# OFA-Sys/OFASys

Hardware: AMD Instinct MI355X
Metric: multimodal tokens/sec (enc+dec train step) (higher is better)
Workload: dtype bf16

## Files before the change

### ofasys_amd/csrc/gemm_mfma.hip

```cpp
#include <mutex>
#include <utility>
#include <vector>

#include "gemm_core.h"

namespace ofa {


#ifdef OFA_GEMM_TIMELINE
#define OFA_TL(i) do { if (threadIdx.x == 0 && (i) < 24) tl[i] = __builtin_amdgcn_s_memtime(); } while (0)
#define OFA_TL_BEGIN                                                                                                           \
  unsigned long long* tl = (unsigned long long*)ws + 32 * (blockIdx.x + gridDim.x * (blockIdx.y + gridDim.y * blockIdx.z));   \
  int tlk = 8;                                                                                                                 \
  if (threadIdx.x == 0) {                                                                                                      \
    tl[5] = __builtin_amdgcn_s_getreg((31 << 11) | 4);                                                                         \
    tl[6] = __builtin_amdgcn_s_getreg((31 << 11) | 20);                                                                        \
    tl[7] = __builtin_amdgcn_s_memrealtime();                                                                                  \
  }                                                                                                                            \
  OFA_TL(0)
#define OFA_TL_STEP do { OFA_TL(tlk); ++tlk; } while (0)
#define OFA_TL_END                                                        \
  do {                                                                    \
    OFA_TL(3);                                                            \
    asm volatile("s_waitcnt vmcnt(0)" ::: "memory");                      \
// ... 229 lines not shown
  const int tid = threadIdx.x, lane = tid & 63, wave = tid >> 6;
  const int wm = wave / WN, wn = wave % WN;
  const int ntiles = tiles_m * tiles_n;
  int t, ks;
  tile_and_slice(ntiles, t, ks);
  constexpr int GM = 8;
  const int gsz = GM * tiles_n;
  const int gid = t / gsz, first_m = gid * GM;
  const int rows_in_group = (tiles_m - first_m) < GM ? (tiles_m - first_m) : GM;
  const int tm = first_m + (t % gsz) % rows_in_group, tn = (t % gsz) / rows_in_group;
  const int m0 = tm * BM, n0 = tn * BN;
  const int bz = blockIdx.z;
  const bf16_t* A = (const bf16_t*)g.A + batch_off(bz, g.batch_inner, g.strideA, g.strideA2);
  const bf16_t* B = (const bf16_t*)g.B + batch_off(bz, g.batch_inner, g.strideB, g.strideB2);
  const int kbeg = ks * ksplit;
  const int kend = (kbeg + ksplit < g.K) ? kbeg + ksplit : g.K;
  const int nk = (kend - kbeg) / BK;

  f32x16 acc[TMW][TNW];
#pragma unroll
  for (int i = 0; i < TMW; ++i)
#pragma unroll
    for (int j = 0; j < TNW; ++j)
#pragma unroll
      for (int r = 0; r < 16; ++r) acc[i][j][r] = 0.f;

  const int wave_u = __builtin_amdgcn_readfirstlane(wave);
  const bf16_t* pa[NVA];
  const bf16_t* pb[NVB];
  glds_ptrs<BM, A_KMAJ, NT, NVA, true>(pa, A, g.lda, m0, g.M, kbeg, tid, g.a_krows);
  glds_ptrs<BN, B_KMAJ, NT, NVB>(pb, B, g.ldb, n0, g.N, kbeg, tid, g.b_krows);
  const int64_t stepA = A_KMAJ ? BK : (int64_t)BK * g.lda, stepB = B_KMAJ ? BK : (int64_t)BK * g.ldb;
  int knext = kbeg;
  auto dma = [&](int stage) {
    if (!A_KMAJ && knext + BK > g.a_krows)
      glds_ptrs<BM, A_KMAJ, NT, NVA, true>(pa, A, g.lda, m0, g.M, knext, tid, g.a_krows);
    if (!B_KMAJ && knext + BK > g.b_krows)
      glds_ptrs<BN, B_KMAJ, NT, NVB>(pb, B, g.ldb, n0, g.N, knext, tid, g.b_krows);
    bf16_t* st = reinterpret_cast<bf16_t*>(smem_raw + (size_t)stage * STG);
    glds_issue<NT, NVA>(pa, stepA, st, wave_u);
    glds_issue<NT, NVB>(pb, stepB, st + EA, wave_u);
    knext += BK;
  };
  int issued = 0;
  for (; issued < S - 1 && issued < nk; ++issued) dma(issued);

  const uint32_t lds0 = (uint32_t)(uintptr_t)smem_raw;
  FragAddr<BM, A_KMAJ> fax[TMW];
  FragAddr<BN, B_KMAJ> faw[TNW];
#pragma unroll
  for (int i = 0; i < TMW; ++i) fax[i].init(lds0, wm * 32 * TMW + i * 32, lane);
#pragma unroll
  for (int j = 0; j < TNW; ++j) faw[j].init(lds0 + (uint32_t)EA * 2u, wn * 32 * TNW + j * 32, lane);
  constexpr int NA = A_KMAJ ? 4 : 1, NB = B_KMAJ ? 4 : 1;
  int stage = 0;
  for (int kt = 0; kt < nk; ++kt) {
    const int later = issued - kt - 1;
    if (S >= 4 && later >= 2) asm volatile("s_waitcnt vmcnt(%0)" ::"n"(2 * P) : "memory");
    else if (later >= 1) asm volatile("s_waitcnt vmcnt(%0)" ::"n"(P) : "memory");
    else asm volatile("s_waitcnt vmcnt(0)" ::: "memory");
    __builtin_amdgcn_sched_barrier(0);
    __builtin_amdgcn_s_barrier();
    __builtin_amdgcn_sched_barrier(0);
    const bool refill = issued < nk;
    bf16_t* rst = reinterpret_cast<bf16_t*>(smem_raw + (size_t)((stage + S - 1) % S) * STG);
    if (refill && !A_KMAJ && knext + BK > g.a_krows)
      glds_ptrs<BM, A_KMAJ, NT, NVA, true>(pa, A, g.lda, m0, g.M, knext, tid, g.a_krows);
    if (refill && !B_KMAJ && knext + BK > g.b_krows)
      glds_ptrs<BN, B_KMAJ, NT, NVB>(pb, B, g.ldb, n0, g.N, knext, tid, g.b_krows);
    u64x2 x0[TMW], w0[TNW], x1[TMW], w1[TNW];
#define RING_ISSUE(KK, X, W)                                                                                           \
    static_for<0, TMW>([&](auto ic) { frag_issue<BM, A_KMAJ, KK, 0>(X[decltype(ic)::value], fax[decltype(ic)::value]); }); \
    static_for<0, TNW>([&](auto jc) { frag_issue<BN, B_KMAJ, KK, 0>(W[decltype(jc)::value], faw[decltype(jc)::value]); })
#define RING_WAIT(X, W)                                                                                                \
    if constexpr (TMW == 2 && TNW == 2) asm volatile("s_waitcnt lgkmcnt(0)" : "+v"(X[0]), "+v"(X[TMW - 1]), "+v"(W[0]), "+v"(W[TNW - 1])); \
    else if constexpr (TMW == 1 && TNW == 2) asm volatile("s_waitcnt lgkmcnt(0)" : "+v"(X[0]), "+v"(W[0]), "+v"(W[TNW - 1]));            \
    else if constexpr (TMW == 2 && TNW == 1) asm volatile("s_waitcnt lgkmcnt(0)" : "+v"(X[0]), "+v"(X[TMW - 1]), "+v"(W[0]));            \
    else { static_assert(TMW <= 2 && TNW <= 2, "RING_WAIT names every fragment register: add the shape");              \
           asm volatile("s_waitcnt lgkmcnt(0)" : "+v"(X[0]), "+v"(W[0])); }
#define RING_MMA(X, W)                                                                                                 \
    _Pragma("unroll") for (int i = 0; i < TMW; ++i) _Pragma("unroll") for (int j = 0; j < TNW; ++j)                    \
        acc[i][j] = mfma16<F16>(W[j], X[i], acc[i][j])
#define RING_DMA(Q)                                                                                                    \
    __builtin_amdgcn_sched_barrier(0);                                                                                 \
    if (refill) {                                                                                                      \
      static_for<(Q) * P / 4, ((Q) + 1) * P / 4>([&](auto pc) {                                                        \
        constexpr int pi = decltype(pc)::value;                                                                        \
        if constexpr (pi < NVA) {                                                                                      \
          __builtin_amdgcn_global_load_lds((gvoid_t*)pa[pi], (lvoid_t*)(rst + (wave_u * 64 + pi * NT) * 8), 16, 0, 0); \
          pa[pi] += stepA;                                                                                             \
        } else {                                                                                                       \
          __builtin_amdgcn_global_load_lds((gvoid_t*)pb[pi - NVA], (lvoid_t*)(rst + EA + (wave_u * 64 + (pi - NVA) * NT) * 8), 16, 0, 0); \
          pb[pi - NVA] += stepB;                                                                                       \
        }                                                                                                              \
      });                                                                                                              \
    }                                                                                                                  \
    __builtin_amdgcn_sched_barrier(0)
    RING_ISSUE(0, x0, w0);
    RING_WAIT(x0, w0);
    RING_ISSUE(1, x1, w1);
    RING_MMA(x0, w0);
    RING_DMA(0);
    RING_WAIT(x1, w1);
    RING_ISSUE(2, x0, w0);
    RING_MMA(x1, w1);
    RING_DMA(1);
    RING_WAIT(x0, w0);
    RING_ISSUE(3, x1, w1);
    RING_MMA(x0, w0);
    RING_DMA(2);
    RING_WAIT(x1, w1);
    RING_MMA(x1, w1);
    RING_DMA(3);
    if (refill) {
      knext += BK;
      ++issued;
    }
#undef RING_DMA
#undef RING_ISSUE
#undef RING_WAIT
#undef RING_MMA
    const bool wrap = stage == S - 1;
    const uint32_t delta = wrap ? (uint32_t)(0u - (uint32_t)(S - 1) * STG) : STG;
#pragma unroll
    for (int i = 0; i < TMW; ++i)
#pragma unroll
      for (int q = 0; q < NA; ++q) fax[i].a[q] += delta;
#pragma unroll
    for (int j = 0; j < TNW; ++j)
#pragma unroll
      for (int q = 0; q < NB; ++q) faw[j].a[q] += delta;
    stage = wrap ? 0 : stage + 1;
  }
  __syncthreads();
  {
    const bool split = gridDim.y > 1;
    constexpr int REGION = ((int)(S * STG) / (WM * WN)) & ~1023;
    unsigned char* wl = smem_raw + wave * REGION;
    const int m_w = m0 + wm * 32 * TMW, n_w = n0 + wn * 32 * TNW;
    if (split) {
      const int64_t n4 = (g.N + 3) & ~3;
      float* wsb = ws + ((int64_t)bz * gridDim.y + ks) * g.M * n4;
      epilogue_lds<TMW, TNW, true, true, F16>(g, acc, wl, REGION, wsb, n4, m_w, n_w, lane);
    } else {
      const int64_t coff = batch_off(bz, g.batch_inner, g.strideC, g.strideC2);
      void* Cb = OUT_F32 ? (void*)((float*)g.C + coff) : (void*)((bf16_t*)g.C + coff);
      epilogue_lds<TMW, TNW, OUT_F32, false, F16>(g, acc, wl, REGION, Cb, g.ldc, m_w, n_w, lane);
    }
  }
}



template <int TM, int TN, bool A_KMAJ, bool B_KMAJ, bool OUT_F32, int WGM, int WGN, bool F16>
__device__ __forceinline__ void gemm_big_body(const GemmArgs& g, int tiles_m, int tiles_n, int ksplit,
                                              float* __restrict__ ws, int t, int ks, int bz, int nsplit, bool to_ws) {
  constexpr int BM = 32 * TM * WGM, BN = 32 * TN * WGN, NT = 64 * WGM * WGN;
  static_assert(BM <= 256 && BN <= 256, "operand stage is 256 rows");
  static_assert(A_KMAJ || BM == 256, "m-major tiles are 256 wide (swizzle)");
  static_assert(B_KMAJ || BN == 256, "m-major tiles are 256 wide (swizzle)");
  constexpr int NVA = BM * 8 / NT, NVB = BN * 8 / NT;
  constexpr int STAGE = 256 * BK;
  extern __shared__ __attribute__((aligned(16))) unsigned char smem_raw[];
  bf16_t* sA0 = reinterpret_cast<bf16_t*>(smem_raw);
  bf16_t* sA1 = sA0 + STAGE;
  bf16_t* sB0 = sA1 + STAGE;
  bf16_t* sB1 = sB0 + STAGE;

  const int tid = threadIdx.x, lane = tid & 63, wave = tid >> 6;
  const int wm = wave / WGN, wn = wave % WGN;
  OFA_TL_BEGIN;
  constexpr int GM = 8;
  const int gsz = GM * tiles_n;
  const int gid = t / gsz, first_m = gid * GM;
  const int rows_in_group = (tiles_m - first_m) < GM ? (tiles_m - first_m) : GM;
  const int tm = first_m + (t % gsz) % rows_in_group, tn = (t % gsz) / rows_in_group;
  const int m0 = tm * BM, n0 = tn * BN;
  const bf16_t* A = (const bf16_t*)g.A + batch_off(bz, g.batch_inner, g.strideA, g.strideA2);
  const bf16_t* B = (const bf16_t*)g.B + batch_off(bz, g.batch_inner, g.strideB, g.strideB2);
  const int kbeg = ks * ksplit;
  const int kend = (kbeg + ksplit < g.K) ? kbeg + ksplit : g.K;
  const int nk = (kend - kbeg) / BK;

  f32x16 acc[TM][TN];
#pragma unroll
  for (int i = 0; i < TM; ++i)
#pragma unroll
    for (int j = 0; j < TN; ++j)
#pragma unroll
      for (int r = 0; r < 16; ++r) acc[i][j][r] = 0.f;

  const int wave_u = __builtin_amdgcn_readfirstlane(wave);
  const bf16_t* pa[NVA];
  const bf16_t* pb[NVB];
  glds_ptrs<BM, A_KMAJ, NT, NVA, true>(pa, A, g.lda, m0, g.M, kbeg, tid, g.a_krows);
  glds_ptrs<BN, B_KMAJ, NT, NVB>(pb, B, g.ldb, n0, g.N, kbeg, tid, g.b_krows);
  const int64_t stepA = A_KMAJ ? BK : (int64_t)BK * g.lda, stepB = B_KMAJ ? BK : (int64_t)BK * g.ldb;
  int knext = kbeg;
  auto dma = [&](bf16_t* da, bf16_t* db) {
    if (!A_KMAJ && knext + BK > g.a_krows)
      glds_ptrs<BM, A_KMAJ, NT, NVA, true>(pa, A, g.lda, m0, g.M, knext, tid, g.a_krows);
    if (!B_KMAJ && knext + BK > g.b_krows)
      glds_ptrs<BN, B_KMAJ, NT, NVB>(pb, B, g.ldb, n0, g.N, knext, tid, g.b_krows);
    glds_issue<NT, NVA>(pa, stepA, da, wave_u);
    glds_issue<NT, NVB>(pb, stepB, db, wave_u);
    knext += BK;
  };
  const uint32_t lds0 = (uint32_t)(uintptr_t)smem_raw;
  BigAddr<BM, A_KMAJ> fax;
  BigAddr<BN, B_KMAJ> faw;
  fax.init(lds0, wm * TM * 32, lane);
  faw.init(lds0 + 2 * STAGE * 2, wn * TN * 32, lane);

  u64x2 xa[2][TM], wb[2][TN];
#ifndef OFA_BIG_RPG_TN
#define OFA_BIG_RPG_TN 1
#endif
  constexpr int RPG = (!A_KMAJ && !B_KMAJ) ? OFA_BIG_RPG_TN : 1;
#define BIG_ISSUE(KK, SET)                                                                                        \
  static_for<0, TM>([&](auto ic) { big_frag<BM, A_KMAJ, KK, decltype(ic)::value, 0>(xa[SET][decltype(ic)::value], fax); }); \
  static_for<0, TN>([&](auto ic) { big_frag<BN, B_KMAJ, KK, decltype(ic)::value, 0>(wb[SET][decltype(ic)::value], faw); })
#define BIG_WAITCNT "s_waitcnt lgkmcnt(0)"
#define BIG_WAIT(SET)                                                                  \
  if constexpr (TM == 4 && TN == 2)                                                    \
    asm volatile(BIG_WAITCNT : "+v"(xa[SET][0]), "+v"(xa[SET][1]), "+v"(xa[SET][2]), "+v"(xa[SET][3]),   \
                 "+v"(wb[SET][0]), "+v"(wb[SET][TN - 1]));                                                          \
  else if constexpr (TM == 3 && TN == 2)                                               \
    asm volatile(BIG_WAITCNT : "+v"(xa[SET][0]), "+v"(xa[SET][1]), "+v"(xa[SET][2]),                     \
                 "+v"(wb[SET][0]), "+v"(wb[SET][TN - 1]));                                                          \
  else if constexpr (TM == 4 && TN == 4)                                               \
    asm volatile(BIG_WAITCNT : "+v"(xa[SET][0]), "+v"(xa[SET][1]), "+v"(xa[SET][2]), "+v"(xa[SET][3]),   \
                 "+v"(wb[SET][0]), "+v"(wb[SET][1]), "+v"(wb[SET][2]), "+v"(wb[SET][TN - 1]));                      \
  else                                                                                 \
    static_assert(TM == 4 && TN == 2, "BIG_WAIT names every fragment register: add the shape")
#define BIG_SB __builtin_amdgcn_sched_barrier(0)
#define BIG_SLICE(SET, KKN)                                                                                         \
  static_for<0, TM * TN>([&](auto tc) {                                                                             \
    constexpr int t = decltype(tc)::value, i = t / TN, j = t % TN;                                                  \
    acc[i][j] = mfma16<F16>(wb[SET][j], xa[SET][i], acc[i][j]); \
    static_for<0, RPG>([&](auto qc) {                                                                               \
      constexpr int r = big_read_after(t * RPG + decltype(qc)::value, TM + TN);                                     \
      if constexpr (r >= 0 && r < TM) big_frag<BM, A_KMAJ, KKN, (r < TM ? r : 0), 0>(xa[1 - (SET)][r < TM ? r : 0], fax); \
      if constexpr (r >= TM) big_frag<BN, B_KMAJ, KKN, (r >= TM ? r - TM : 0), 0>(wb[1 - (SET)][r >= TM ? r - TM : 0], faw); \
    });                                                                                                             \
    BIG_SB;                                                                                                         \
  })
  if (nk > 0) {
    dma(sA0, sB0);
    asm volatile("s_waitcnt vmcnt(0)" ::: "memory");
    __syncthreads();
    OFA_TL(1);
    if (nk > 1) dma(sA1, sB1);
    BIG_ISSUE(0, 0);
    bf16_t* curA = sA0;
    bf16_t* curB = sB0;
    for (int kt = 0; kt < nk; ++kt) {
      BIG_WAIT(0); BIG_SB; BIG_SLICE(0, 1);
      BIG_WAIT(1); BIG_SB; BIG_SLICE(1, 2);
      BIG_WAIT(0); BIG_SB; BIG_SLICE(0, 3);
      BIG_WAIT(1);
      if (kt + 1 < nk) {
        asm volatile("s_waitcnt vmcnt(0)" ::: "memory");
        __syncthreads();
      }
      const bool more2 = kt + 2 < nk;
      if (more2 && !A_KMAJ && knext + BK > g.a_krows)
        glds_ptrs<BM, A_KMAJ, NT, NVA, true>(pa, A, g.lda, m0, g.M, knext, tid, g.a_krows);
      if (more2 && !B_KMAJ && knext + BK > g.b_krows)
        glds_ptrs<BN, B_KMAJ, NT, NVB>(pb, B, g.ldb, n0, g.N, knext, tid, g.b_krows);
#pragma unroll
      for (int i = 0; i < 4; ++i) {
        fax.a[i] ^= (uint32_t)(STAGE * 2);
        faw.a[i] ^= (uint32_t)(STAGE * 2);
      }
      BIG_SB;
      static_for<0, TM * TN>([&](auto tc) {
        constexpr int t = decltype(tc)::value, i = t / TN, j = t % TN;
        acc[i][j] = mfma16<F16>(wb[1][j], xa[1][i], acc[i][j]);
        static_for<0, RPG>([&](auto qc) {
          constexpr int r = big_read_after(t * RPG + decltype(qc)::value, TM + TN);
          if constexpr (r >= 0 && r < TM) big_frag<BM, A_KMAJ, 0, (r < TM ? r : 0), 0>(xa[0][r < TM ? r : 0], fax);
          if constexpr (r >= TM) big_frag<BN, B_KMAJ, 0, (r >= TM ? r - TM : 0), 0>(wb[0][r >= TM ? r - TM : 0], faw);
        });
        if (more2) {
          constexpr int NP = NVA + NVB, NM = TM * TN;
          static_for<t * NP / NM, (t + 1) * NP / NM>([&](auto pc) {
            constexpr int pi = decltype(pc)::value;
            if constexpr (pi < NVA) {
              __builtin_amdgcn_global_load_lds((gvoid_t*)pa[pi], (lvoid_t*)(curA + (wave_u * 64 + pi * NT) * 8), 16, 0, 0);
              pa[pi] += stepA;
            } else {
              __builtin_amdgcn_global_load_lds((gvoid_t*)pb[pi - NVA], (lvoid_t*)(curB + (wave_u * 64 + (pi - NVA) * NT) * 8), 16, 0, 0);
              pb[pi - NVA] += stepB;
            }
          });
        }
        BIG_SB;
      });
      if (more2) knext += BK;
      OFA_TL_STEP;
      curA = (bf16_t*)((uintptr_t)curA ^ (uintptr_t)(STAGE * 2));
      curB = (bf16_t*)((uintptr_t)curB ^ (uintptr_t)(STAGE * 2));
    }
    BIG_WAIT(0);
  }
#undef BIG_SLICE
#undef BIG_SB
#undef BIG_WAIT
#undef BIG_ISSUE
  __syncthreads();
  OFA_TL(2);
  {
    const bool split = to_ws || nsplit > 1;
    constexpr int REGION = 4 * STAGE * 2 / (WGM * WGN);
    unsigned char* wl = smem_raw + wave * REGION;
    const int m_w = m0 + wm * TM * 32, n_w = n0 + wn * TN * 32;
    if (split) {
      const int64_t n4 = (g.N + 3) & ~3;
      float* wsb = ws + ((int64_t)bz * nsplit + ks) * g.M * n4;
      epilogue_lds<TM, TN, true, true, F16>(g, acc, wl, REGION, wsb, n4, m_w, n_w, lane);
    } else {
      const int64_t coff = batch_off(bz, g.batch_inner, g.strideC, g.strideC2);
      void* Cb = OUT_F32 ? (void*)((float*)g.C + coff) : (void*)((bf16_t*)g.C + coff);
      epilogue_lds<TM, TN, OUT_F32, false, F16>(g, acc, wl, REGION, Cb, g.ldc, m_w, n_w, lane);
    }
  }
  OFA_TL_END;
}

template <int TM, int TN, bool A_KMAJ, bool B_KMAJ, bool OUT_F32, int WGM = 2, int WGN = 2, bool F16 = false>
__global__ __launch_bounds__(64 * WGM * WGN) void gemm_big_kernel(GemmArgs g, int tiles_m, int tiles_n, int ksplit,
                                                                 float* __restrict__ ws) {
  int t, ks;
  tile_and_slice(tiles_m * tiles_n, t, ks);
  gemm_big_body<TM, TN, A_KMAJ, B_KMAJ, OUT_F32, WGM, WGN, F16>(g, tiles_m, tiles_n, ksplit, ws, t, ks, (int)blockIdx.z,
                                                                (int)gridDim.y, false);
}

template <bool B_KMAJ, bool OUT_F32, bool F16>
__global__ __launch_bounds__(512) void gemm_big_mixed_kernel(GemmArgs g, int tiles_n, int rows_big, int rows_small) {
  const int nbig = rows_big * tiles_n, nsmall = rows_small * tiles_n;
  const int xcd = blockIdx.x & 7, local = blockIdx.x >> 3;
  auto lo = [](int n, int x) { const int q = n >> 3, r = n & 7; return x < r ? x * (q + 1) : r * (q + 1) + (x - r) * q; };
  const int b0 = lo(nbig, xcd), nb = lo(nbig, xcd + 1) - b0, s0 = lo(nsmall, xcd), ns = lo(nsmall, xcd + 1) - s0;
  if (local < nb) {
    gemm_big_body<4, 2, true, B_KMAJ, OUT_F32, 2, 4, F16>(g, rows_big, tiles_n, g.K, nullptr, b0 + local, 0, 0, 1, false);
  } else if (local - nb < ns) {
    const int64_t r0 = (int64_t)rows_big * 256;
    g.A = (const bf16_t*)g.A + r0 * g.lda;
    g.C = OUT_F32 ? (void*)((float*)g.C + r0 * g.ldc) : (void*)((bf16_t*)g.C + r0 * g.ldc);
    g.M -= (int)r0;
    gemm_big_body<3, 2, true, B_KMAJ, OUT_F32, 2, 4, F16>(g, rows_small, tiles_n, g.K, nullptr, s0 + local - nb, 0, 0, 1, false);
  }
}

struct TileTime {
  int slots;
  double step, step_nt, per_tile;
  double tile_us(int nk, bool nt) const { return nk * (nt ? step_nt : step) + per_tile; }
  double us(int64_t tiles, int nk, bool nt) const { return (double)cdiv(tiles, slots) * tile_us(nk, nt); }
};
constexpr TileTime TT_128{512, 0.90, 1.0, 4.2}, TT_256{256, 1.45, 1.45, 7.6}, TT_192{256, 1.13, 1.13, 6.5};

static double mixed_time_us(int nbig, int nsmall, int nk) {
  const double t4 = TT_256.tile_us(nk, false), t3 = TT_192.tile_us(nk, false);
  double worst = 0.0;
  for (int x = 0; x < 8; ++x) {
    auto lo = [](int n, int x_) { const int q = n >> 3, r = n & 7; return x_ < r ? x_ * (q + 1) : r * (q + 1) + (x_ - r) * q; };
    const int nb = lo(nbig, x + 1) - lo(nbig, x), ns = lo(nsmall, x + 1) - lo(nsmall, x);
    double cu[32];
    for (int c = 0; c < 32; ++c) cu[c] = 0.0;
    for (int i = 0; i < nb + ns; ++i) {
      int best = 0;
      for (int c = 1; c < 32; ++c) best = cu[c] < cu[best] ? c : best;
      cu[best] += i < nb ? t4 : t3;
    }
    for (int c = 0; c < 32; ++c) worst = cu[c] > worst ? cu[c] : worst;
  }
  return worst;
}

constexpr int BIG_LDS = 4 * 256 * BK * sizeof(bf16_t);

bool gemm_lds_attr(const void* kern, int bytes, uint64_t& done) {
  int dev = 0;
  if (hipGetDevice(&dev) != hipSuccess || dev < 0 || dev >= 64) return false;
  if (done >> dev & 1) return true;
  if (hipFuncSetAttribute(kern, hipFuncAttributeMaxDynamicSharedMemorySize, bytes) != hipSuccess) {
    (void)hipGetLastError();
    return false;
  }
  done |= 1ull << dev;
  return true;
}

template <bool BKM, bool OF, bool F16>
static bool launch_big_mixed(const GemmArgs& g, int rows_big, int rows_small, hipStream_t st) {
  const int tiles_n = cdiv(g.N, 256), nbig = rows_big * tiles_n, nsmall = rows_small * tiles_n;
  auto kern = gemm_big_mixed_kernel<BKM, OF, F16>;
  static uint64_t attr_done = 0;
  if (!gemm_lds_attr((const void*)kern, BIG_LDS, attr_done)) return false;
  const int per_xcd = cdiv(nbig, 8) + cdiv(nsmall, 8);
  hipLaunchKernelGGL(kern, dim3(8 * per_xcd), dim3(512), BIG_LDS, st, g, tiles_n, rows_big, rows_small);
  return true;
}


template <bool F16, bool = false>
__global__ __launch_bounds__(512) void gemm_group_tn_kernel(GroupArgs ga) {
  GemmArgs g;
  int t, ks;
  const GroupItem* itp = group_enter(ga, g, t, ks);
  if (!itp) return;
  const GroupItem& it = *itp;
  gemm_big_body<4, 2, false, false, false, 2, 4, F16>(g, it.tiles_m, it.tiles_n, it.ksplit, it.ws, t, ks, 0, it.splits, it.out == nullptr);
}

template <bool OUT_F32, bool F16 = false>
__global__ __launch_bounds__(256) void splitk_reduce_kernel(GemmArgs g, const float* __restrict__ ws, int splits) {
  const int64_t quads = (int64_t)g.M * ((g.N + 3) / 4);
  const int bz = blockIdx.y;
  const int64_t coff = batch_off(bz, g.batch_inner, g.strideC, g.strideC2);
  void* Cb = OUT_F32 ? (void*)((float*)g.C + coff) : (void*)((bf16_t*)g.C + coff);
  for (int64_t i = (int64_t)blockIdx.x * blockDim.x + threadIdx.x; i < quads; i += (int64_t)gridDim.x * blockDim.x) {
    const int m = (int)(i / ((g.N + 3) / 4)), n = (int)(i % ((g.N + 3) / 4)) * 4;
    float4 s = make_float4(0.f, 0.f, 0.f, 0.f);
    for (int k = 0; k < splits; ++k) {
      const float4 p = *reinterpret_cast<const float4*>(ws + (((int64_t)bz * splits + k) * g.M + m) * ((g.N + 3) & ~3) + n);
      s.x += p.x; s.y += p.y; s.z += p.z; s.w += p.w;
    }
    epilogue_store<OUT_F32, F16>(g, Cb, m, n, s.x, s.y, s.z, s.w);
  }
}

bool gemm_mfma_supported(const GemmArgs& g) {
  if (g.M <= 0 || g.N <= 0 || g.K <= 0) return false;
  const int64_t M8 = (g.M + 7) & ~7, N8 = (g.N + 7) & ~7, N4 = (g.N + 3) & ~3, K8 = (g.K + 7) & ~7;
  if ((g.lda & 7) || (g.ldb & 7) || (g.ldc & 3) || N4 > g.ldc) return false;
  if ((g.strideA & 7) || (g.strideB & 7) || (g.strideC & 3)) return false;
  if ((g.strideA2 & 7) || (g.strideB2 & 7) || (g.strideC2 & 3)) return false;
  if (!g.transA && (g.K & 7)) {
    if (g.transB || !(g.flags & OFA_GEMM_A_KPAD_ZERO) || K8 > g.lda) return false;
  }
  if (g.transB && (g.K & 7)) return false;
  if (g.transA && M8 > g.lda) return false;
  if (!g.transB && N8 > g.ldb) return false;
  if ((g.flags & OFA_GEMM_BIAS_COL) && (g.N & 3)) return false;
  if (((uintptr_t)g.A & 15) || ((uintptr_t)g.B & 15) || ((uintptr_t)g.C & 15)) return false;
  if ((g.flags & OFA_GEMM_BIAS_COL) && ((uintptr_t)g.bias & 7)) return false;
  return true;
}

struct GemmPlan {
  int kernel;
  int wm, wn;
  int tm, tn;
  int splits, ksplit, K;
  int mixed_a, mixed_b;
  int colstat_rows;
  bool reduce;
  int pp;
  int bm() const { return 32 * tm * wm; }
  int bn() const { return 32 * tn * wn; }
};

struct PlanKnobs {
  int tile = 0;
  int pp = -1;
  int mixed = -1;
  int split_min_k = 2048;
};

static PlanKnobs plan_knobs() {
  PlanKnobs k;
#ifdef OFA_DEBUG_SWITCHES
  auto env = [](const char* name, int dflt) { const char* e = getenv(name); return e ? atoi(e) : dflt; };
  static const int split_min_k = env("OFA_GEMM_SPLIT_MIN_K", k.split_min_k);
  k = PlanKnobs{env("OFA_GEMM_TILE", k.tile), env("OFA_GEMM_PP", k.pp), env("OFA_GEMM_MIXED", k.mixed), split_min_k};
#endif
  return k;
}

static int pp_variant(const PlanKnobs& kn, bool trans_a, bool trans_b, int K) {
  if (kn.pp >= 0) return kn.pp;
  if (trans_a && !trans_b) return 23;
  if (!trans_a && !trans_b && K >= 2048) return 23;
  return 0;
}

static GemmPlan gemm_plan(GemmArgs g, int batch, bool has_ws, int64_t ws_bytes, const PlanKnobs& kn) {
  if ((g.flags & OFA_GEMM_A_KPAD_ZERO) && !g.transA && !g.transB && (g.K % BK) != 0 && ((g.K + BK - 1) / BK) * BK <= g.lda)
    g.K = ((g.K + BK - 1) / BK) * BK;
  if (g.transA && !g.transB && (g.K % BK) != 0 && !(g.flags & OFA_GEMM_NO_LDS_DMA)) g.K = ((g.K + BK - 1) / BK) * BK;
  const bool dma = (g.K % BK) == 0 && !(g.flags & OFA_GEMM_NO_LDS_DMA);
  const int64_t t22 = (int64_t)cdiv(g.M, 128) * cdiv(g.N, 128) * batch;
  const int64_t t12 = (int64_t)cdiv(g.M, 64) * cdiv(g.N, 128) * batch;
  const int64_t t11 = (int64_t)cdiv(g.M, 64) * cdiv(g.N, 64) * batch;
  int maxs = has_ws ? g.K / 256 : 1;
  maxs = maxs < 1 ? 1 : (maxs > 32 ? 32 : maxs);
  if (g.K < kn.split_min_k || t22 >= 256) maxs = 1;
  if (!g.transA && g.K <= 4096 && t11 >= 256) maxs = 1;
  const int64_t want = 384;
  int wm, wn;
  int64_t tiles;
  if (t22 * maxs >= want && g.M > 64 && g.N >= 128) { wm = 2; wn = 2; tiles = t22; }
  else if (t12 * maxs >= want && g.N >= 128) { wm = 1; wn = 2; tiles = t12; }
  else { wm = 1; wn = 1; tiles = t11; }
  if (kn.tile == 22) { wm = 2; wn = 2; tiles = t22; }
  else if (kn.tile == 12) { wm = 1; wn = 2; tiles = t12; }
  else if (kn.tile == 11) { wm = 1; wn = 1; tiles = t11; }
  int big_tm = 0;
  const bool big_ok = dma && g.N >= 256 && g.M >= 192;
  const bool forced_small = kn.tile == 22 || kn.tile == 12 || kn.tile == 11;
  const int nk = g.K / BK;
  const int64_t t4 = (int64_t)cdiv(g.M, 256) * cdiv(g.N, 256) * batch, t3 = (int64_t)cdiv(g.M, 192) * cdiv(g.N, 256) * batch;
  if (big_ok && !forced_small) {
    if (kn.tile == 44 || kn.tile == 84) big_tm = 4;
    else if (kn.tile == 34 || kn.tile == 83) big_tm = g.transA ? 4 : 3;
    else if (!g.transA) {
      if (batch == 1 && nk >= 4 && t22 >= 512 && wm == 2 && wn == 2) {
        const double e2 = TT_128.us(t22, nk, g.transB);
        const double e4 = t4 >= 128 ? TT_256.us(t4, nk, false) : 1e30, e3 = t3 >= 128 ? TT_192.us(t3, nk, false) : 1e30;
        if (e4 <= e3 && e4 < 0.95 * e2) big_tm = 4;
        else if (e3 < e4 && e3 < 0.95 * e2) big_tm = 3;
      }
    } else {
      const double f4 = (double)t4 / (double)(cdiv(t4, 256) * 256) * ((double)g.M / (cdiv(g.M, 256) * 256)) * ((double)g.N / (cdiv(g.N, 256) * 256));
      if (f4 >= 0.7 && (g.K >= 1024 || t4 <= 256)) big_tm = 4;
    }
    if (big_tm) tiles = big_tm == 4 ? t4 : t3;
  }
  int splits = 1;
  if (!big_tm && big_ok && !kn.tile && !g.transA && batch == 1 && has_ws && g.K >= 8192) {
    int s = t4 <= 64 ? (int)(256 / t4) : 1;
    s = s > maxs ? maxs : s;
    while (s > 1 && (int64_t)s * g.M * ((g.N + 3) & ~3) * 4 > ws_bytes) --s;
    if (s >= 4) {
      big_tm = 4;
      tiles = t4;
      splits = s;
    }
  }
  if (!big_tm && tiles < want && maxs > 1) {
    splits = (int)((want + tiles - 1) / tiles);
    if (splits > maxs) splits = maxs;
    while (splits > 1 && (int64_t)splits * batch * g.M * ((g.N + 3) & ~3) * 4 > ws_bytes) --splits;
  }
  int ksplit = g.K;
  if (splits > 1) {
    ksplit = cdiv(cdiv(g.K, splits), BK) * BK;
    splits = cdiv(g.K, ksplit);
  }
  GemmPlan p{};
  p.splits = splits;
  p.ksplit = ksplit;
  p.K = g.K;
  p.reduce = splits > 1 && !(g.flags & OFA_GEMM_DEFER_REDUCE);
  if (big_tm) {
    p.wm = 2; p.wn = 4; p.tm = big_tm; p.tn = 2;
    p.pp = pp_variant(kn, g.transA, g.transB, g.K);
    p.kernel = p.pp && !(g.flags & OFA_GEMM_OUT_F32) && !(g.transA && g.transB) ? OFA_GEMM_KERNEL_PP : OFA_GEMM_KERNEL_BIG;
  } else if (dma && (int64_t)cdiv(g.M, 64 * wm) * cdiv(g.N, 64 * wn) * splits * batch <= ((wm == 1 && wn == 1) ? 512 : 256) &&
             ksplit >= 4 * BK) {
    p.kernel = OFA_GEMM_KERNEL_RING;
    p.wm = 2; p.wn = 2; p.tm = wm; p.tn = wn;
  } else {
    p.kernel = dma ? OFA_GEMM_KERNEL_LDS_DMA : OFA_GEMM_KERNEL_REG;
    p.wm = wm; p.wn = wn; p.tm = 2; p.tn = 2;
  }
  p.colstat_rows = splits > 1 || batch != 1 ? 0 : 32 * p.tm;
  if (kn.mixed != 0 && big_ok && !kn.tile && !g.transA && batch == 1 && splits == 1 && !g.colstat && !(g.flags & OFA_GEMM_BIAS_ROW) &&
      g.M >= 1024 && g.N >= 512 && g.K >= 4 * BK && pp_variant(kn, false, g.transB != 0, g.K) == 0) {
    struct Key { int M, N, K, tb; };
    struct Val { int a, b; double t; };
    static std::mutex mu;
    static std::vector<std::pair<Key, Val>> cache;
    const int tiles_n = cdiv(g.N, 256);
    Val best{0, 0, 1e30};
    bool hit = false;
    {
      std::lock_guard<std::mutex> lk(mu);
      for (auto& e : cache)
        if (e.first.M == g.M && e.first.N == g.N && e.first.K == g.K && e.first.tb == g.transB) { best = e.second; hit = true; break; }
    }
    if (!hit) {
      const int amax = g.M / 256;
      for (int a = 1; a <= amax; ++a) {
        const int rest = g.M - a * 256;
        if (rest <= 0) break;
        const int b = cdiv(rest, 192);
        const double t = mixed_time_us(a * tiles_n, b * tiles_n, nk);
        if (t < best.t) best = Val{a, b, t};
      }
      std::lock_guard<std::mutex> lk(mu);
      if (cache.size() < 256) cache.push_back({Key{g.M, g.N, g.K, g.transB}, best});
    }
    const bool modelled = (wm == 2 && wn == 2) || big_tm;
    const double cur = big_tm == 4 ? TT_256.us(tiles, nk, false) : big_tm == 3 ? TT_192.us(tiles, nk, false) : TT_128.us(tiles, nk, g.transB);
    if (best.a > 0 && best.b > 0 && (kn.mixed == 1 || (modelled && best.t < 0.95 * cur))) {
      p.kernel = OFA_GEMM_KERNEL_MIXED;
      p.wm = 2; p.wn = 4; p.tm = 4; p.tn = 2;
      p.mixed_a = best.a;
      p.mixed_b = best.b;
    }
  }
  return p;
}

template <auto KERN>
static void launch_tiles(int lds, const GemmArgs& g, int batch, const GemmPlan& p, float* ws, hipStream_t st) {
  static uint64_t attr_done = 0;
  (void)gemm_lds_attr((const void*)KERN, lds, attr_done);
  const int tiles_m = cdiv(g.M, p.bm()), tiles_n = cdiv(g.N, p.bn());
  hipLaunchKernelGGL(KERN, dim3(tiles_m * tiles_n, p.splits, batch), dim3(64 * p.wm * p.wn), lds, st, g, tiles_m, tiles_n, p.ksplit, ws);
}

template <int WM, int WN, bool AK, bool BKM, bool OF, bool F16>
static void launch_cfg2(const GemmArgs& g, int batch, const GemmPlan& p, float* ws, hipStream_t st) {
  constexpr int BM = 64 * WM, BN = 64 * WN;
  if (p.kernel == OFA_GEMM_KERNEL_LDS_DMA)
    launch_tiles<gemm_mfma_kernel<WM, WN, AK, BKM, OF, true, F16>>(2 * (BM + BN) * BK * sizeof(bf16_t), g, batch, p, ws, st);
  else
    launch_tiles<gemm_mfma_kernel<WM, WN, AK, BKM, OF, false, F16>>(2 * (TileGeom<BM, AK>::ELEMS + TileGeom<BN, BKM>::ELEMS) * sizeof(bf16_t),
                                                                    g, batch, p, ws, st);
}

template <bool AK, bool BKM, bool OF, bool F16>
static int launch_plan(const GemmArgs& g, int batch, const GemmPlan& p, float* ws, hipStream_t st) {
  switch (p.kernel) {
    case OFA_GEMM_KERNEL_PP:
      if (gemm_pp_launch(p.pp, g, batch, p.tm, p.splits, p.ksplit, ws, st, F16)) break;
      [[fallthrough]];
    case OFA_GEMM_KERNEL_BIG:
      if constexpr (AK) {
        if (p.tm == 3) { launch_tiles<gemm_big_kernel<3, 2, AK, BKM, OF, 2, 4, F16>>(BIG_LDS, g, batch, p, ws, st); break; }
      }
      launch_tiles<gemm_big_kernel<4, 2, AK, BKM, OF, 2, 4, F16>>(BIG_LDS, g, batch, p, ws, st);
      break;
    case OFA_GEMM_KERNEL_RING: {
      const int lds = 4 * (p.bm() + p.bn()) * BK * sizeof(bf16_t);
      if (p.tm == 1 && p.tn == 1) launch_tiles<gemm_ring_kernel<2, 2, AK, BKM, OF, 4, F16, 1, 1>>(lds, g, batch, p, ws, st);
      else if (p.tm == 1) launch_tiles<gemm_ring_kernel<2, 2, AK, BKM, OF, 4, F16, 1, 2>>(lds, g, batch, p, ws, st);
      else launch_tiles<gemm_ring_kernel<2, 2, AK, BKM, OF, 4, F16, 2, 2>>(lds, g, batch, p, ws, st);
      break;
    }
    default:
      if (p.wm == 2) launch_cfg2<2, 2, AK, BKM, OF, F16>(g, batch, p, ws, st);
      else if (p.wn == 2) launch_cfg2<1, 2, AK, BKM, OF, F16>(g, batch, p, ws, st);
      else launch_cfg2<1, 1, AK, BKM, OF, F16>(g, batch, p, ws, st);
  }
  int rc = check_launch("gemm_mfma");
  if (rc || !p.reduce) return rc;
  const int64_t quads = (int64_t)g.M * ((g.N + 3) / 4);
  dim3 grid((unsigned)((quads + 255) / 256 > 2048 ? 2048 : (quads + 255) / 256), batch), block(256);
  hipLaunchKernelGGL((splitk_reduce_kernel<OF, F16>), grid, block, 0, st, g, (const float*)ws, p.splits);
  return check_launch("gemm_splitk_reduce");
}

int gemm_mfma_launch(const GemmArgs& g_in, int batch, void* ws, int64_t ws_bytes, hipStream_t st, bool f16) {
  const PlanKnobs kn = plan_knobs();
  GemmPlan p = gemm_plan(g_in, batch, ws != nullptr, ws_bytes, kn);
  GemmArgs g = g_in;
  g.a_krows = g.b_krows = g.K;
  g.K = p.K;
  if (g.colstat) g.colstat_rows = p.colstat_rows;
  if (p.kernel == OFA_GEMM_KERNEL_MIXED) {
    if (with_layout(g, f16, [&](auto, auto bk, auto of, auto h) { return launch_big_mixed<bk, of, h>(g, p.mixed_a, p.mixed_b, st); }))
      return check_launch("gemm_big_mixed");
    p = gemm_plan(g_in, batch, ws != nullptr, ws_bytes, PlanKnobs{kn.tile, kn.pp, 0, kn.split_min_k});
  }
  return with_layout(g, f16, [&](auto ak, auto bk, auto of, auto h) { return launch_plan<ak, bk, of, h>(g, batch, p, (float*)ws, st); });
}

static int gemm_mfma_colstat_groups(const GemmArgs& g, void* ws, int64_t ws_bytes) {
  if ((g.flags & (OFA_GEMM_OUT_F32 | OFA_GEMM_ACCUM)) || (g.N & 7)) return 0;
  const int rows = gemm_plan(g, 1, ws != nullptr, ws_bytes, plan_knobs()).colstat_rows;
  return rows ? cdiv(g.M, rows) : 0;
}

static GemmArgs dense_args(int M, int N, int K, int transA, int transB, int flags) {
  GemmArgs g{};
  g.M = M; g.N = N; g.K = K; g.transA = transA; g.transB = transB; g.flags = flags;
  g.lda = transA ? M : K; g.ldb = transB ? K : N; g.ldc = N;
  return g;
}

}

using namespace ofa;

extern "C" int ofa_gemm_splits(int M, int N, int K, int transA, int transB, int batch, int flags, int dtype, int64_t ws_bytes) {
  if ((dtype != OFA_BF16 && dtype != OFA_F16) || (flags & OFA_GEMM_FORCE_SIMPLE) || M <= 0 || N <= 0 || K <= 0 || batch <= 0) return 1;
  return gemm_plan(dense_args(M, N, K, transA, transB, flags), batch, ws_bytes > 0, ws_bytes, plan_knobs()).splits;
}

extern "C" int ofa_gemm_plan(int M, int N, int K, int transA, int transB, int batch, int flags, int dtype, int64_t ws_bytes, int* plan) {
  OFA_REQUIRE(plan && OFA_DT_OK(dtype) && M > 0 && N > 0 && K > 0 && batch > 0, OFA_ERR_INVALID, "gemm_plan: bad argument");
  memset(plan, 0, OFA_GEMM_PLAN_LEN * sizeof(int));
  const GemmArgs g = dense_args(M, N, K, transA, transB, flags);
  const int why = dtype == OFA_F32 ? 1 : (flags & OFA_GEMM_FORCE_SIMPLE) ? 2 : !gemm_mfma_supported(g) ? 3 : 0;
  if (why) { plan[OFA_GEMM_PLAN_SIMPLE_WHY] = why; return 0; }
  const GemmPlan p = gemm_plan(g, batch, ws_bytes > 0, ws_bytes, plan_knobs());
  const int v[] = {p.kernel, 0, p.wm, p.wn, p.tm, p.tn, p.bm(), p.bn(), p.splits, p.ksplit, p.K, p.mixed_a, p.mixed_b, p.colstat_rows, p.reduce};
  static_assert(sizeof(v) / sizeof(v[0]) == OFA_GEMM_PLAN_LEN, "one value per plan field");
  memcpy(plan, v, sizeof(v));
  return 0;
}

static bool group_item_ok(const ofa_gemm_group_item& it) {
  if (it.m <= 0 || it.n <= 0 || it.k <= 0 || !it.a || !it.b) return false;
  if ((it.m & 7) || (it.n & 7)) return false;
  if (it.lda < it.m || it.ldb < it.n || (it.lda & 7) || (it.ldb & 7)) return false;
  if (((uintptr_t)it.a & 15) || ((uintptr_t)it.b & 15)) return false;
  return true;
}

static double group_time_us(const ofa_gemm_group_item* items, int n, int len) {
  int steps[GROUP_MAX], count[GROUP_MAX], total = 0;
  double slab_bytes = 0.0;
  for (int p = 0; p < n; ++p) {
    int sp = cdiv(items[p].k, len);
    sp = sp > 32 ? 32 : sp;
    const int ksplit = cdiv(cdiv(items[p].k, BK), sp) * BK;
    sp = cdiv(items[p].k, ksplit);
    steps[p] = ksplit / BK;
    count[p] = cdiv(items[p].m, 256) * cdiv(items[p].n, 256) * sp;
    total += count[p];
    if (sp > 1) slab_bytes += ((double)sp * 4.0 + 4.0) * items[p].m * items[p].n;
  }
  double worst = 0.0;
  for (int x = 0; x < 8; ++x) {
    const int q = total >> 3, r = total & 7;
    const int lo = x < r ? x * (q + 1) : r * (q + 1) + (x - r) * q, hi = lo + q + (x < r ? 1 : 0);
    double cu[32];
    for (int c = 0; c < 32; ++c) cu[c] = 0.0;
    int id = 0;
    for (int p = 0; p < n; ++p)
      for (int w = 0; w < count[p]; ++w, ++id) {
        if (id < lo || id >= hi) continue;
        int best = 0;
        for (int c = 1; c < 32; ++c) best = cu[c] < cu[best] ? c : best;
        cu[best] += 1.5 * steps[p] + 6.0;
      }
    for (int c = 0; c < 32; ++c) worst = cu[c] > worst ? cu[c] : worst;
  }
  return worst + (slab_bytes > 0.0 ? 2.0 + slab_bytes / 4.1e6 : 0.0);
}

static int group_plan_len(const ofa_gemm_group_item* items, int n);
static void group_plan(ofa_gemm_group_item* items, int n) {
  struct Key { int n; int mnk[GROUP_MAX][3]; };
  static std::mutex mu;
  static std::vector<std::pair<Key, int>> cache;
  Key key{};
  key.n = n;
  for (int p = 0; p < n; ++p) { key.mnk[p][0] = items[p].m; key.mnk[p][1] = items[p].n; key.mnk[p][2] = items[p].k; }
  int len = -1;
  {
    std::lock_guard<std::mutex> lk(mu);
    for (auto& e : cache)
      if (!memcmp(&e.first, &key, sizeof(Key))) { len = e.second; break; }
  }
  if (len < 0) {
    len = group_plan_len(items, n);
    std::lock_guard<std::mutex> lk(mu);
    if (cache.size() < 512) cache.push_back({key, len});
  }
  for (int p = 0; p < n; ++p) {
    int sp = cdiv(items[p].k, len);
    sp = sp > 32 ? 32 : sp;
    const int ksplit = cdiv(cdiv(items[p].k, BK), sp) * BK;
    items[p].splits = cdiv(items[p].k, ksplit);
  }
}

static int group_plan_len(const ofa_gemm_group_item* items, int n) {
  int kmax = 0;
  for (int p = 0; p < n; ++p) kmax = items[p].k > kmax ? items[p].k : kmax;
  const int tiles = cdiv(kmax, BK);
  int len = tiles * BK;
  double best = group_time_us(items, n, len);
  for (int sp = 2; sp <= 32 && cdiv(tiles, sp) >= 4; ++sp) {
    const int l = cdiv(tiles, sp) * BK;
    const double t = group_time_us(items, n, l);
    if (t < best * 0.97) { best = t; len = l; }
  }
  return len;
}
// ... 92 lines not shown
```

Baseline: 1.421 million.

## Use three-stage A operand ring in big GEMM kernel for tm=3 k-major tiles

Adds an A3 variant of the big MFMA GEMM body that keeps three LDS stages for the A operand while B stays double-buffered. A is prefetched two k-steps ahead, and the per-iteration wait becomes a partial vmcnt, so the barrier no longer waits on the newest A loads. The launcher picks this variant for the tm=3 k-major path when the larger dynamic LDS allocation can be set, and otherwise falls back. It needs more LDS per block, which may lower occupancy, and adds ring-index bookkeeping.

Measured after the change: 1.427 million (median of 6 runs). About the same (+0.4%).

```diff
diff --git a/ofasys_amd/csrc/gemm_mfma.hip b/ofasys_amd/csrc/gemm_mfma.hip
--- a/ofasys_amd/csrc/gemm_mfma.hip
+++ b/ofasys_amd/csrc/gemm_mfma.hip
@@ -405,7 +405,7 @@
 
 
 
-template <int TM, int TN, bool A_KMAJ, bool B_KMAJ, bool OUT_F32, int WGM, int WGN, bool F16>
+template <int TM, int TN, bool A_KMAJ, bool B_KMAJ, bool OUT_F32, int WGM, int WGN, bool F16, bool A3 = false>
 __device__ __forceinline__ void gemm_big_body(const GemmArgs& g, int tiles_m, int tiles_n, int ksplit,
                                               float* __restrict__ ws, int t, int ks, int bz, int nsplit, bool to_ws) {
   constexpr int BM = 32 * TM * WGM, BN = 32 * TN * WGN, NT = 64 * WGM * WGN;
@@ -414,10 +414,12 @@
   static_assert(B_KMAJ || BN == 256, "m-major tiles are 256 wide (swizzle)");
   constexpr int NVA = BM * 8 / NT, NVB = BN * 8 / NT;
   constexpr int STAGE = 256 * BK;
+  static_assert(!A3 || A_KMAJ, "the three-stage A ring is built for a k-major A (its DMA never re-derives pointers at a ragged tail)");
+  static_assert(!A3 || NVA <= 63, "vmcnt field");
   extern __shared__ __attribute__((aligned(16))) unsigned char smem_raw[];
-  bf16_t* sA0 = reinterpret_cast<bf16_t*>(smem_raw);
+  bf16_t* sA0 = reinterpret_cast<bf16_t*>(smem_raw) + (A3 ? 2 * STAGE : 0);
   bf16_t* sA1 = sA0 + STAGE;
-  bf16_t* sB0 = sA1 + STAGE;
+  bf16_t* sB0 = reinterpret_cast<bf16_t*>(smem_raw) + (A3 ? 0 : 2 * STAGE);
   bf16_t* sB1 = sB0 + STAGE;
 
   const int tid = threadIdx.x, lane = tid & 63, wave = tid >> 6;
@@ -462,8 +464,8 @@
   const uint32_t lds0 = (uint32_t)(uintptr_t)smem_raw;
   BigAddr<BM, A_KMAJ> fax;
   BigAddr<BN, B_KMAJ> faw;
-  fax.init(lds0, wm * TM * 32, lane);
-  faw.init(lds0 + 2 * STAGE * 2, wn * TN * 32, lane);
+  fax.init(lds0 + (A3 ? 2 * STAGE * 2 : 0), wm * TM * 32, lane);
+  faw.init(lds0 + (A3 ? 0 : 2 * STAGE * 2), wn * TN * 32, lane);
 
   u64x2 xa[2][TM], wb[2][TN];
 #ifndef OFA_BIG_RPG_TN
@@ -504,26 +506,41 @@
     __syncthreads();
     OFA_TL(1);
     if (nk > 1) dma(sA1, sB1);
+    if constexpr (A3) {
+      if (nk > 2) glds_issue<NT, NVA>(pa, stepA, sA0 + 2 * STAGE, wave_u);
+    }
     BIG_ISSUE(0, 0);
     bf16_t* curA = sA0;
     bf16_t* curB = sB0;
+    int sa = 0;
     for (int kt = 0; kt < nk; ++kt) {
       BIG_WAIT(0); BIG_SB; BIG_SLICE(0, 1);
       BIG_WAIT(1); BIG_SB; BIG_SLICE(1, 2);
       BIG_WAIT(0); BIG_SB; BIG_SLICE(0, 3);
       BIG_WAIT(1);
       if (kt + 1 < nk) {
-        asm volatile("s_waitcnt vmcnt(0)" ::: "memory");
-        __syncthreads();
+        if constexpr (A3) {
+          if (kt + 2 < nk) asm volatile("s_waitcnt vmcnt(%0)" ::"n"(NVA) : "memory");
+          else asm volatile("s_waitcnt vmcnt(0)" ::: "memory");
+          BIG_SB;
+          __builtin_amdgcn_s_barrier();
+          BIG_SB;
+        } else {
+          asm volatile("s_waitcnt vmcnt(0)" ::: "memory");
+          __syncthreads();
+        }
       }
       const bool more2 = kt + 2 < nk;
+      const bool moreA = A3 ? kt + 3 < nk : more2;
       if (more2 && !A_KMAJ && knext + BK > g.a_krows)
         glds_ptrs<BM, A_KMAJ, NT, NVA, true>(pa, A, g.lda, m0, g.M, knext, tid, g.a_krows);
       if (more2 && !B_KMAJ && knext + BK > g.b_krows)
         glds_ptrs<BN, B_KMAJ, NT, NVB>(pb, B, g.ldb, n0, g.N, knext, tid, g.b_krows);
+      const uint32_t stepa = sa == 2 ? (uint32_t)(0u - 2u * (uint32_t)(STAGE * 2)) : (uint32_t)(STAGE * 2);
 #pragma unroll
       for (int i = 0; i < 4; ++i) {
-        fax.a[i] ^= (uint32_t)(STAGE * 2);
+        if constexpr (A3) fax.a[i] += stepa;
+        else fax.a[i] ^= (uint32_t)(STAGE * 2);
         faw.a[i] ^= (uint32_t)(STAGE * 2);
       }
       BIG_SB;
@@ -535,7 +552,23 @@
           if constexpr (r >= 0 && r < TM) big_frag<BM, A_KMAJ, 0, (r < TM ? r : 0), 0>(xa[0][r < TM ? r : 0], fax);
           if constexpr (r >= TM) big_frag<BN, B_KMAJ, 0, (r >= TM ? r - TM : 0), 0>(wb[0][r >= TM ? r - TM : 0], faw);
         });
-        if (more2) {
+        if constexpr (A3) {
+          constexpr int NP = NVA + NVB, NM = TM * TN;
+          static_for<t * NP / NM, (t + 1) * NP / NM>([&](auto pc) {
+            constexpr int pi = decltype(pc)::value;
+            if constexpr (pi < NVB) {
+              if (more2) {
+                __builtin_amdgcn_global_load_lds((gvoid_t*)pb[pi], (lvoid_t*)(curB + (wave_u * 64 + pi * NT) * 8), 16, 0, 0);
+                pb[pi] += stepB;
+              }
+            } else {
+              if (moreA) {
+                __builtin_amdgcn_global_load_lds((gvoid_t*)pa[pi - NVB], (lvoid_t*)(curA + (wave_u * 64 + (pi - NVB) * NT) * 8), 16, 0, 0);
+                pa[pi - NVB] += stepA;
+              }
+            }
+          });
+        } else if (more2) {
           constexpr int NP = NVA + NVB, NM = TM * TN;
           static_for<t * NP / NM, (t + 1) * NP / NM>([&](auto pc) {
             constexpr int pi = decltype(pc)::value;
@@ -552,7 +585,12 @@
       });
       if (more2) knext += BK;
       OFA_TL_STEP;
-      curA = (bf16_t*)((uintptr_t)curA ^ (uintptr_t)(STAGE * 2));
+      if constexpr (A3) {
+        sa = sa == 2 ? 0 : sa + 1;
+        curA = sA0 + sa * STAGE;
+      } else {
+        curA = (bf16_t*)((uintptr_t)curA ^ (uintptr_t)(STAGE * 2));
+      }
       curB = (bf16_t*)((uintptr_t)curB ^ (uintptr_t)(STAGE * 2));
     }
     BIG_WAIT(0);
@@ -581,13 +619,13 @@
   OFA_TL_END;
 }
 
-template <int TM, int TN, bool A_KMAJ, bool B_KMAJ, bool OUT_F32, int WGM = 2, int WGN = 2, bool F16 = false>
+template <int TM, int TN, bool A_KMAJ, bool B_KMAJ, bool OUT_F32, int WGM = 2, int WGN = 2, bool F16 = false, bool A3 = false>
 __global__ __launch_bounds__(64 * WGM * WGN) void gemm_big_kernel(GemmArgs g, int tiles_m, int tiles_n, int ksplit,
                                                                  float* __restrict__ ws) {
   int t, ks;
   tile_and_slice(tiles_m * tiles_n, t, ks);
-  gemm_big_body<TM, TN, A_KMAJ, B_KMAJ, OUT_F32, WGM, WGN, F16>(g, tiles_m, tiles_n, ksplit, ws, t, ks, (int)blockIdx.z,
-                                                                (int)gridDim.y, false);
+  gemm_big_body<TM, TN, A_KMAJ, B_KMAJ, OUT_F32, WGM, WGN, F16, A3>(g, tiles_m, tiles_n, ksplit, ws, t, ks, (int)blockIdx.z,
+                                                                    (int)gridDim.y, false);
 }
 
 template <bool B_KMAJ, bool OUT_F32, bool F16>
@@ -634,6 +672,14 @@
 }
 
 constexpr int BIG_LDS = 4 * 256 * BK * sizeof(bf16_t);
+constexpr int BIG_LDS_A3 = 5 * 256 * BK * sizeof(bf16_t);
+
+static bool big_three_a_stages() {
+#ifdef OFA_DEBUG_SWITCHES
+  if (const char* e = getenv("OFA_PREFETCH_OLD")) return !(atoi(e) & 1);
+#endif
+  return true;
+}
 
 bool gemm_lds_attr(const void* kern, int bytes, uint64_t& done) {
   int dev = 0;
@@ -886,7 +932,14 @@
       [[fallthrough]];
     case OFA_GEMM_KERNEL_BIG:
       if constexpr (AK) {
-        if (p.tm == 3) { launch_tiles<gemm_big_kernel<3, 2, AK, BKM, OF, 2, 4, F16>>(BIG_LDS, g, batch, p, ws, st); break; }
+        if (p.tm == 3) {
+          static uint64_t ok3 = 0;
+          if (big_three_a_stages() && gemm_lds_attr((const void*)gemm_big_kernel<3, 2, AK, BKM, OF, 2, 4, F16, true>, BIG_LDS_A3, ok3))
+            launch_tiles<gemm_big_kernel<3, 2, AK, BKM, OF, 2, 4, F16, true>>(BIG_LDS_A3, g, batch, p, ws, st);
+          else
+            launch_tiles<gemm_big_kernel<3, 2, AK, BKM, OF, 2, 4, F16>>(BIG_LDS, g, batch, p, ws, st);
+          break;
+        }
       }
       launch_tiles<gemm_big_kernel<4, 2, AK, BKM, OF, 2, 4, F16>>(BIG_LDS, g, batch, p, ws, st);
       break;
```
